# totgokhung123/Event-Retrival-In-Video-Learning-Transferable-Visual-Model-From-Supervised-Natural-Language

Hardware: AMD Instinct MI355X
Metric: frames/sec embedded+ranked, ViT-B/32 224², 1/2/4/8 MI355X; R@1/5/10 parity (higher is better)
Workload: dtype bf16; 1 GPU; ViT-B/32 bf16, 10000 frames/GPU x 32 text queries, top-10 (BASELINE configs[1]); frames_per_gpu=10000, global_frames=10000, queries=32, k=10, image_chunk=10000, parallelism=dp1

## Files before the change

### event-retrival-in-video-learning-transferable-visual-model-from-supervised-natural-language_amd/csrc/api.cpp

```cpp
#include <hip/hip_runtime.h>

#include <cmath>
#include <cstdarg>
#include <cstdlib>
#include <cstdio>
#include <cstring>
#include <algorithm>
#include <functional>
#include <memory>
#include <mutex>
#include <string>
#include <system_error>
#include <thread>
#include <vector>

#include "../../include/miclip.h"
#include "src_hash.h"
#include "internal.hpp"

using namespace miclip;

namespace {

thread_local std::string g_err;
// ... 628 lines not shown
    HIP_TRY(gemm_bf16(with_variant(gargs(c->h, W, L.w_qkv, W, L.b_qkv, c->qkv, 3 * W, M, 3 * W, W), GV_QKV), EPI_BF16,
                      s));
    HIP_TRY(attention(c->qkv, c->att, B, S, W, causal, s));
    HIP_TRY(gemm_bf16(with_variant(gargs(c->att, W, L.w_out, W, L.b_out, c->delta, W, M, W, W), GV_OUT), EPI_BF16, s));
    HIP_TRY(residual_ln(c->x, c->delta, W, 1, L.ln2_g, L.ln2_b, c->h, M, W, s, nullptr, nullptr, xmode_at(r16, l)));
    HIP_TRY(gemm_bf16(with_variant(gargs(c->h, W, L.w_fc, W, L.b_fc, c->mlp, 4 * W, M, 4 * W, W), GV_FC),
                      EPI_GELU_BF16, s));
    HIP_TRY(gemm_bf16(with_variant(gargs(c->mlp, 4 * W, L.w_proj, 4 * W, L.b_proj, c->delta, W, M, W, 4 * W), GV_PROJ),
                      EPI_BF16, s));
    if (l + 1 < layers.size())
      HIP_TRY(residual_ln(c->x, c->delta, W, 1, layers[l + 1].ln1_g, layers[l + 1].ln1_b, c->h, M, W, s, nullptr, nullptr,
                          r16 ? 2 : 0));
  }
  return MI_OK;
}

static int lnfold(int W) { return ab_env_int("MICLIP_LNFOLD", W <= 1024) != 0; }

static GemmArgs ln_args(mi_clip* c, const uint16_t* wf, const float* sv, const float* cv, void* out, int N, int M,
                        int W) {
  GemmArgs g = gargs((const uint16_t*)c->x, 2 * W, wf, W, cv, out, N, M, N, W);
  g.variant = 0;
  g.a_f16 = 1;
  g.rs = c->rs;
  g.colv = sv;
  return g;
}

static int resfuse() { return ab_env_int("MICLIP_RESFUSE", 1) != 0; }

struct Carve {
  char* base;
  size_t cap, off = 0, end = 0;
  void* take(size_t bytes) {
    char* p = base + off;
    end = off + bytes;
    off = (end + 255) & ~(size_t)255;
    return p;
  }
  int fits(const char* what) const {
    return end <= cap ? MI_OK : fail(MI_ERR_ARG, "%s: %zu bytes needed, %zu reserved", what, end, cap);
  }
};
struct ClsRows { void* att; uint8_t* sc; float* x; };
struct RowsOut { char* out; int dtype, l2; };

static int borrow_h(mi_clip* c, size_t bytes, float** p) {
  Carve h{(char*)c->h, c->h_bytes};
  *p = (float*)h.take(bytes);
  return h.fits("rows borrowed from the h buffer");
}

static int gather_rows(void* dst, size_t dst_pitch, const void* src, size_t src_pitch, size_t bytes_per_row, int B,
                       hipStream_t s) {
  HIP_TRY(hipMemcpy2DAsync(dst, dst_pitch, src, src_pitch, bytes_per_row, B, hipMemcpyDeviceToDevice, s));
  return MI_OK;
}

static int gemm_residual(mi_clip* c, const uint16_t* A, int64_t lda, const uint16_t* w, const float* b, float* x, int M,
                         int W, int K, hipStream_t s) {
  GemmArgs g = gargs(A, lda, w, K, b, x, 2 * W, M, W, K);
  MI_TRY(borrow_h(c, (size_t)M * (W / 64) * 8, &g.ps));
  HIP_TRY(gemm_bf16(g, EPI_RES16_BF16, s));
  HIP_TRY(residual_finalize(g.ps, c->rs, M, W, s));
  return MI_OK;
}

static int cls_last() { return ab_env_int("MICLIP_CLS_LAST", 1) != 0; }
static bool cls_att_compact(int S) { return S <= 64 && ab_env_int("MICLIP_CLS_ATT", 1) != 0; }

static bool cls_rows(bool last_layer, int B, int S, bool pre) {
  return last_layer && pre && B >= 256 && S > 1 && cls_last();
}

static int cls_gather(mi_clip* c, int B, int S, int W, const void* att, size_t att_row, const uint8_t* att_sc,
                      size_t x_bytes, hipStream_t s, ClsRows* r, float** xpost, int64_t* post_stride) {
  Carve q{(char*)c->qkv, c->qkv_bytes};
  r->att = q.take(B * att_row);
  r->sc = (uint8_t*)q.take(att_sc ? ((size_t)W / 128) * (B + 2) * 2 : 0);
  r->x = (float*)q.take((size_t)B * W * 4);
  MI_TRY(q.fits("the last block's CLS rows in the qkv buffer"));
  if (att) MI_TRY(gather_rows(r->att, att_row, att, S * att_row, att_row, B, s));
  if (att_sc) {
    const size_t mp = ((size_t)B * S + 1) & ~(size_t)1, bp = ((size_t)B + 1) & ~(size_t)1;
    for (int st = 0; st < W / 128; ++st)
      MI_TRY(gather_rows(r->sc + st * bp * 2, 2, att_sc + st * mp * 2, (size_t)S * 2, 2, B, s));
  }
  MI_TRY(gather_rows(r->x, (size_t)W * 4, c->x, (size_t)S * W * 4, x_bytes, B, s));
  *xpost = r->x;
  *post_stride = 1;
  return MI_OK;
}

using InProjArgs = std::function<GemmArgs(int n0, int N, int rows, int64_t stride)>;
static int in_proj_cls(mi_clip* c, int B, int S, int W, const float* vec, size_t vec_row, const float* GemmArgs::*f,
                       int epi, hipStream_t s, const InProjArgs& mk) {
  float* vec_c;
  MI_TRY(borrow_h(c, B * vec_row, &vec_c));
  HIP_TRY(gemm_bf16(mk(W, 2 * W, B * S, 1), epi, s));
  MI_TRY(gather_rows(vec_c, vec_row, vec, S * vec_row, vec_row, B, s));
  GemmArgs q = mk(0, W, B, S);
  q.*f = vec_c;
  HIP_TRY(gemm_bf16(q, epi, s));
  return MI_OK;
}

static int last_block_cls(mi_clip* c, const Layer& L, int B, int S, int W, bool att_compact, float** xpost,
                          int64_t* post_stride, hipStream_t s) {
  ClsRows r;
  MI_TRY(cls_gather(c, B, S, W, att_compact ? nullptr : c->att, (size_t)W * 2, nullptr, (size_t)W * 2, s, &r, xpost,
                    post_stride));
  if (att_compact) r.att = c->att;
  MI_TRY(gemm_residual(c, (const uint16_t*)r.att, W, L.w_out, L.b_out, r.x, B, W, W, s));
  GemmArgs f = ln_args(c, L.lw_fc, L.ls_fc, L.lc_fc, c->mlp, 4 * W, B, W);
  f.A = (const uint16_t*)r.x;
  HIP_TRY(gemm_bf16(f, EPI_LN_GELU_BF16, s));
  HIP_TRY(gemm_bf16(with_variant(gargs(c->mlp, 4 * W, L.w_proj, 4 * W, L.b_proj, c->delta, W, B, W, 4 * W), GV_PROJ),
                    EPI_BF16, s));
  return MI_OK;
}

static int run_tower_fold(mi_clip* c, const std::vector<Layer>& layers, int B, int S, int W, hipStream_t s,
                          float** xpost, int64_t* post_stride) {
  const int M = B * S;
  const bool fuse = resfuse() && !gemm_variant_for(GV_OUT) && !gemm_variant_for(GV_PROJ) && !gemm_variant();
  *xpost = c->x;
  *post_stride = S;
  for (size_t l = 0; l < layers.size(); ++l) {
    const Layer& L = layers[l];
    const bool last = l + 1 == layers.size();
    const bool cls = cls_rows(last, B, S, fuse);
    auto in_proj = [&](int n0, int N, int rows, int64_t stride) {
      GemmArgs g = ln_args(c, L.lw_qkv + (size_t)n0 * W, L.ls_qkv + n0, L.lc_qkv + n0, c->qkv + n0, N, rows, W);
      g.lda = stride * 2 * W;
      g.ldo = stride * 3 * W;
      return g;
    };
    if (cls) MI_TRY(in_proj_cls(c, B, S, W, c->rs, 8, &GemmArgs::rs, EPI_LN_BF16, s, in_proj));
    else HIP_TRY(gemm_bf16(in_proj(0, 3 * W, M, 1), EPI_LN_BF16, s));
// ... 586 lines not shown
  int r = check_rank_args(N, D, corpus_dtype, Q, 1, norm_mode, MI_NAN_FIRST);
  if (r) return r;
  if (N == 0 || Q == 0) return MI_OK;
  if (!corpus || !queries || !out) return fail(MI_ERR_ARG, "mi_score_matrix: null pointer");
  HIP_TRY(score_matrix(corpus, N, D, corpus_dtype, queries, Q, norm_mode, out, (hipStream_t)stream));
  return MI_OK;
}

int mi_rank_of_targets(const float* scores, int64_t Q, int64_t N, const int64_t* pq, const int64_t* pt, int64_t T,
                       int64_t* out, void* stream) {
  if (Q < 0 || N < 0 || T < 0) return fail(MI_ERR_ARG, "negative size");
  if (T == 0) return MI_OK;
  if (!scores || !pq || !pt || !out) return fail(MI_ERR_ARG, "mi_rank_of_targets: null pointer");
  HIP_TRY(rank_of_targets(scores, Q, N, pq, pt, T, out, (hipStream_t)stream));
  return MI_OK;
}

int mi_op_gemm(const void* A, const void* W, const float* bias, void* out, int32_t M, int32_t N, int32_t K,
               int32_t epi, void* stream) {
  if (!A || !W || !out || M < 0) return fail(MI_ERR_ARG, "mi_op_gemm: bad arguments");
  if (K % 64 || N % 128 || K <= 0) return fail(MI_ERR_UNSUPPORTED, "mi_op_gemm: needs K %% 64 == 0, N %% 128 == 0");
  const int variant = epi >> 8;
  if (variant && !MICLIP_AB) return fail(MI_ERR_UNSUPPORTED, "mi_op_gemm: schedule overrides need the A/B build (make ab)");
  epi &= 0xff;
  if (epi < 0 || epi > 3) return fail(MI_ERR_ARG, "mi_op_gemm: bad epilogue");
  GemmArgs g = gargs((const uint16_t*)A, K, (const uint16_t*)W, K, bias, out, N, M, N, K);
  if (variant) g.variant = variant;
  HIP_TRY(gemm_bf16(g, epi, (hipStream_t)stream));
  return MI_OK;
}

int mi_op_gemm_f32(const float* A, const float* W, const float* bias, float* out, int32_t M, int32_t N, int32_t K,
                   int32_t epi, void* stream) {
  if (!A || !W || !out || M < 0 || N < 1) return fail(MI_ERR_ARG, "mi_op_gemm_f32: bad arguments");
  if (K % 32 || K <= 0) return fail(MI_ERR_UNSUPPORTED, "mi_op_gemm_f32: needs K %% 32 == 0");
  static const int epis[4] = {EPI_F32, EPI_GELU_BF16, EPI_RESID_F32, EPI_RELU_F32};
  if (epi < 0 || epi > 3) return fail(MI_ERR_ARG, "mi_op_gemm_f32: epilogue 0 (store), 1 (QuickGELU), 2 (+=), 3 (ReLU)");
  HIP_TRY(gemm_f32(A, K, W, K, bias, out, N, M, N, K, epis[epi], (hipStream_t)stream));
  return MI_OK;
}

extern "C" int mi_debug_gemm_probe(unsigned long long* host, int32_t n) {
  if (!host || n < 0) return fail(MI_ERR_ARG, "mi_debug_gemm_probe: bad arguments");
  HIP_TRY(gemm_probe_read(host, n));
  return MI_OK;
}

extern "C" int mi_debug_gemm8q_probe(unsigned long long* host, int32_t n) {
  if (!host || n < 0) return fail(MI_ERR_ARG, "mi_debug_gemm8q_probe: bad arguments");
  HIP_TRY(gemm8q_probe_read(host, n));
  return MI_OK;
}

int mi_op_layernorm(const float* x, const float* g, const float* b, void* out, int32_t rows, int32_t W,
                    void* stream) {
  if (!x || !g || !b || !out || rows < 0) return fail(MI_ERR_ARG, "mi_op_layernorm: bad arguments");
  if (W % 4 || W > 1024) return fail(MI_ERR_UNSUPPORTED, "mi_op_layernorm: W must be a multiple of 4, <= 1024");
  HIP_TRY(layernorm_bf16(x, W, g, b, (uint16_t*)out, W, rows, W, (hipStream_t)stream));
  return MI_OK;
}

int mi_op_residual_ln(void* x, const void* delta, const float* g, const float* b, void* out, int32_t rows, int32_t W,
                      int32_t xmode, void* stream) {
  if (!x || !delta || !g || !b || !out || rows < 0) return fail(MI_ERR_ARG, "mi_op_residual_ln: bad arguments");
  if (W % 4 || W > 1024) return fail(MI_ERR_UNSUPPORTED, "mi_op_residual_ln: W must be a multiple of 4, <= 1024");
  if (xmode < 0 || xmode > 2) return fail(MI_ERR_ARG, "mi_op_residual_ln: xmode must be 0, 1 or 2");
  HIP_TRY(residual_ln((float*)x, (const uint16_t*)delta, W, 1, g, b, (uint16_t*)out, rows, W, (hipStream_t)stream,
                      nullptr, nullptr, xmode));
  return MI_OK;
}

int mi_op_split6(const float* x, int64_t ldx, int64_t rows, int32_t K, int32_t role, int32_t gelu, void* out,
                 void* stream) {
  if (!x || !out || rows < 0 || (role & ~1) || (gelu & ~1)) return fail(MI_ERR_ARG, "mi_op_split6: bad arguments");
  if (K < 4 || K % 4 || ldx < K || ldx % 4) return fail(MI_ERR_UNSUPPORTED, "mi_op_split6: K %% 4 == 0, ldx >= K, ldx %% 4 == 0");
  HIP_TRY(split6_rows(x, ldx, rows, K, role, gelu, (uint16_t*)out, (hipStream_t)stream));
  return MI_OK;
}

int mi_clip_kernel_events(mi_clip* c, int32_t kind, int32_t capacity) {
  if (!c || kind < 0 || kind > MI_KERNEL_C_FC || capacity < 0 || capacity > (1 << 16))
    return fail(MI_ERR_ARG, "mi_clip_kernel_events: bad arguments");
  std::lock_guard<std::mutex> g(c->mu);
  HIP_TRY(hipSetDevice(c->device));
  while ((int)c->ev.size() < 2 * capacity) {
    hipEvent_t e;
    HIP_TRY(hipEventCreate(&e));
    c->ev.push_back(e);
  }
  c->ev_kind = capacity ? kind : 0;
  c->ev_cap = capacity;
  c->ev_n = 0;
  return MI_OK;
}

int mi_clip_kernel_times(mi_clip* c, float* us, int32_t n) {
  if (!c || (!us && n > 0) || n < 0) return fail(MI_ERR_ARG, "mi_clip_kernel_times: bad arguments");
  std::lock_guard<std::mutex> g(c->mu);
  const int m = c->ev_n < n ? c->ev_n : n;
  for (int i = 0; i < m; ++i) {
    HIP_TRY(hipEventSynchronize(c->ev[2 * i + 1]));
    float ms = 0.f;
    HIP_TRY(hipEventElapsedTime(&ms, c->ev[2 * i], c->ev[2 * i + 1]));
    us[i] = ms * 1e3f;
  }
  return m;
// ... 256 lines not shown
```

### event-retrival-in-video-learning-transferable-visual-model-from-supervised-natural-language_amd/csrc/encoder.hip

```cpp
#include <cstdlib>

#include "common.hpp"
#include "internal.hpp"

namespace miclip {

namespace {

constexpr float LN_EPS = 1e-5f;

struct RowVals {
  float4 v[4];
};

__device__ __forceinline__ void ln_stats(RowVals& r, int n4, int lane, int W, float& mean, float& rstd) {
  float s = 0.f;
#pragma unroll
  for (int i = 0; i < 4; ++i)
    if (lane + 64 * i < n4) s += (r.v[i].x + r.v[i].y) + (r.v[i].z + r.v[i].w);
  mean = wave_sum(s) / (float)W;
  float ss = 0.f;
#pragma unroll
  for (int i = 0; i < 4; ++i)
    if (lane + 64 * i < n4) {
// ... 150 lines not shown
    ln_stats(r, n4, lane, W, mean, rstd);
    ln_store(r, mean, rstd, g1, b1, h + (int64_t)row * W, nullptr, nullptr, row, 0, lane, n4);
  }
}

__device__ __forceinline__ void store_row_stats(RowVals& r, int n4, int lane, int W, float* rs, int row) {
  float mean, rstd;
  ln_stats(r, n4, lane, W, mean, rstd);
  if (lane == 0) *(float2*)(rs + 2 * (int64_t)row) = make_float2(rstd, rstd * mean);
}

__global__ __launch_bounds__(256) void vision_embed_ln16_kernel(float* __restrict__ x, const float* __restrict__ cls,
                                                                const float* __restrict__ pos,
                                                                const float* __restrict__ g,
                                                                const float* __restrict__ b, int rows, int S, int W,
                                                                float* __restrict__ rs) {
  typedef _Float16 h4v __attribute__((ext_vector_type(4)));
  const int row = blockIdx.x * 4 + (threadIdx.x >> 6), lane = threadIdx.x & 63;
  if (row >= rows) return;
  const int t = row % S, n4 = W >> 2;
  const float4* xr = (const float4*)(x + (int64_t)row * W);
  h4v* xh = (h4v*)((_Float16*)x + (int64_t)row * W * 2);
  const float4* src = t == 0 ? (const float4*)cls : xr;
  const float4* p4 = (const float4*)(pos + (int64_t)t * W);
  RowVals r;
#pragma unroll
  for (int i = 0; i < 4; ++i) {
    const int idx = lane + 64 * i;
    if (idx < n4) {
      const float4 sv = src[idx], p = p4[idx];
      r.v[i] = make_float4(sv.x + p.x, sv.y + p.y, sv.z + p.z, sv.w + p.w);
    } else {
      r.v[i] = make_float4(0.f, 0.f, 0.f, 0.f);
    }
  }
  float mean, rstd;
  ln_stats(r, n4, lane, W, mean, rstd);
  const float4* g4 = (const float4*)g;
  const float4* b4 = (const float4*)b;
#pragma unroll
  for (int i = 0; i < 4; ++i) {
    const int idx = lane + 64 * i;
    if (idx < n4) {
      const float4 gg = g4[idx], bb = b4[idx];
      const h4v o{(_Float16)((r.v[i].x - mean) * rstd * gg.x + bb.x), (_Float16)((r.v[i].y - mean) * rstd * gg.y + bb.y),
                  (_Float16)((r.v[i].z - mean) * rstd * gg.z + bb.z), (_Float16)((r.v[i].w - mean) * rstd * gg.w + bb.w)};
      r.v[i] = make_float4((float)o[0], (float)o[1], (float)o[2], (float)o[3]);
      xh[idx] = o;
    }
  }
  store_row_stats(r, n4, lane, W, rs, row);
}

__global__ __launch_bounds__(256) void residual_stats_kernel(float* __restrict__ x, const uint16_t* __restrict__ delta,
                                                             float* __restrict__ rs, int rows, int W) {
  typedef _Float16 h4v __attribute__((ext_vector_type(4)));
  typedef uint32_t u2v __attribute__((ext_vector_type(2)));
  const int row = blockIdx.x * 4 + (threadIdx.x >> 6), lane = threadIdx.x & 63;
  if (row >= rows) return;
  const int n4 = W >> 2;
  h4v* xh = (h4v*)((_Float16*)x + (int64_t)row * W * 2);
  const u2v* dr = (const u2v*)(delta + (int64_t)row * W);
  RowVals r;
#pragma unroll
  for (int i = 0; i < 4; ++i) {
    const int idx = lane + 64 * i;
    if (idx < n4) {
      const h4v vh = __builtin_nontemporal_load(&xh[idx]);
      const u2v d = __builtin_nontemporal_load(&dr[idx]);
      const h4v o{(_Float16)((float)vh[0] + bf2f((uint16_t)(d[0] & 0xffff))),
                  (_Float16)((float)vh[1] + bf2f((uint16_t)(d[0] >> 16))),
                  (_Float16)((float)vh[2] + bf2f((uint16_t)(d[1] & 0xffff))),
                  (_Float16)((float)vh[3] + bf2f((uint16_t)(d[1] >> 16)))};
      __builtin_nontemporal_store(o, &xh[idx]);
      r.v[i] = make_float4((float)o[0], (float)o[1], (float)o[2], (float)o[3]);
    } else {
      r.v[i] = make_float4(0.f, 0.f, 0.f, 0.f);
    }
  }
  store_row_stats(r, n4, lane, W, rs, row);
}

__global__ __launch_bounds__(256) void residual_finalize_kernel(const float* __restrict__ ps, float* __restrict__ rs,
                                                                int rows, int W) {
  __shared__ float4 sp[256 * 8 + 256 / 4];
  const int np = W >> 6, nq = np >> 1;
  const int r0 = blockIdx.x * 256;
  const int nrow = min(256, rows - r0);
  const float4* src = (const float4*)(ps + (int64_t)r0 * np * 2);
  for (int i = threadIdx.x; i < nrow * nq; i += 256) {
    const int r = i / nq;
    sp[i + (r >> 2)] = src[i];
  }
  __syncthreads();
  const int row = r0 + threadIdx.x;
  if (row >= rows) return;
  const float4* p4 = sp + threadIdx.x * nq + (threadIdx.x >> 2);
  float s[16], m2[16];
#pragma unroll
  for (int i = 0; i < 8; ++i)
    if (i < nq) {
      const float4 v = p4[i];
      s[2 * i] = v.x;
      m2[2 * i] = v.y;
      s[2 * i + 1] = v.z;
      m2[2 * i + 1] = v.w;
    }
  float tot = 0.f;
#pragma unroll
  for (int j = 0; j < 16; ++j)
    if (j < np) tot += s[j];
  const float mean = tot / (float)W;
  float acc = 0.f;
#pragma unroll
  for (int j = 0; j < 16; ++j)
    if (j < np) {
      const float dm = s[j] * (1.0f / 64.0f) - mean;
      acc += m2[j] + 64.0f * dm * dm;
    }
  const float rstd = 1.0f / sqrtf(acc / (float)W + LN_EPS);
  *(float2*)(rs + 2 * (int64_t)row) = make_float2(rstd, rstd * mean);
}

__global__ __launch_bounds__(256) void text_embed_kernel(const int32_t* __restrict__ tokens,
                                                         const float* __restrict__ tok_emb,
                                                         const float* __restrict__ pos, float* __restrict__ x,
                                                         int64_t total4, int S, int W, int vocab) {
  const int64_t i = (int64_t)blockIdx.x * 256 + threadIdx.x;
  if (i >= total4) return;
  const int n4 = W >> 2;
  const int64_t row = i / n4;
  const int c = (int)(i % n4);
  const int t = (int)(row % S);
  int tok = tokens[row];
  tok = tok < 0 ? 0 : (tok >= vocab ? vocab - 1 : tok);
  const float4 e = ((const float4*)(tok_emb + (int64_t)tok * W))[c];
  const float4 p = ((const float4*)(pos + (int64_t)t * W))[c];
  ((float4*)x)[i] = make_float4(e.x + p.x, e.y + p.y, e.z + p.z, e.w + p.w);
}

__global__ __launch_bounds__(256) void eot_gather_ln_kernel(const int32_t* __restrict__ tokens,
                                                            const float* __restrict__ x,
                                                            const uint16_t* __restrict__ delta,
                                                            const float* __restrict__ g,
                                                            const float* __restrict__ b, uint16_t* __restrict__ out,
// ... 72 lines not shown

template <bool IN_BF16>
__global__ __launch_bounds__(256) void im2col_kernel(const void* __restrict__ pixels, uint16_t* __restrict__ out,
                                                     int64_t total8, int R, int P, int G, int Kp) {
  const int64_t i = (int64_t)blockIdx.x * 256 + threadIdx.x;
  if (i >= total8) return;
  const int k8 = Kp >> 3;
  const int64_t prow = i / k8;
  const int kb = (int)(i % k8) * 8;
  const int64_t bimg = prow / (G * G);
  const int p = (int)(prow % (G * G));
  const int gy = p / G, gx = p % G;
  const int PP = P * P, K = 3 * PP;
  uint32_t packed[4];
#pragma unroll
  for (int e = 0; e < 8; e += 2) {
    float v[2];
#pragma unroll
    for (int u = 0; u < 2; ++u) {
      const int k = kb + e + u;
      if (k < K) {
        const int c = k / PP, rem = k % PP, kh = rem / P, kw = rem % P;
        const int64_t off = ((bimg * 3 + c) * R + (gy * P + kh)) * (int64_t)R + gx * P + kw;
        v[u] = IN_BF16 ? bf2f(((const uint16_t*)pixels)[off]) : ((const float*)pixels)[off];
      } else {
        v[u] = 0.f;
      }
    }
    packed[e >> 1] = (uint32_t)f2bf(v[0]) | ((uint32_t)f2bf(v[1]) << 16);
  }
  *(uint4*)(out + prow * Kp + kb) = make_uint4(packed[0], packed[1], packed[2], packed[3]);
}

__global__ __launch_bounds__(256) void finalize_kernel(const float* __restrict__ y, void* __restrict__ out,
                                                       int out_dtype, int rows, int D, int l2) {
  const int row = blockIdx.x * 4 + (threadIdx.x >> 6), lane = threadIdx.x & 63;
  if (row >= rows) return;
  const float* yr = y + (int64_t)row * D;
  float inv = 1.f;
  if (l2) {
    float ss = 0.f;
    for (int c = lane; c < D; c += 64) ss += yr[c] * yr[c];
    const float n = sqrtf(wave_sum(ss));
    inv = (l2 == 2 && !(n > 1e-8f)) ? 1.0f : 1.0f / n;
  }
  for (int c = lane; c < D; c += 64) {
    const float v = l2 ? yr[c] * inv : yr[c];
    if (out_dtype == 0) ((float*)out)[(int64_t)row * D + c] = v;
    else if (out_dtype == 1) ((uint16_t*)out)[(int64_t)row * D + c] = f2bf(v);
    else ((_Float16*)out)[(int64_t)row * D + c] = (_Float16)v;
  }
}

}

hipError_t layernorm_bf16(const float* x, int64_t in_stride, const float* g, const float* b, uint16_t* out,
                          int64_t out_stride, int rows, int W, hipStream_t s, uint8_t* q, uint8_t* qs) {
  if (rows <= 0) return hipSuccess;
  if (W % 4 || W > 1024 || (q && W % 128)) return hipErrorInvalidValue;
  hipLaunchKernelGGL(ln_bf16_kernel, dim3((rows + 3) / 4), dim3(256), 0, s, x, in_stride, g, b, out, out_stride,
                     rows, W, q, qs);
  return hipGetLastError();
}

hipError_t vision_embed_ln(float* x, const float* cls, const float* pos, const float* g, const float* b, int B,
                           int S, int W, hipStream_t s, const float* g1, const float* b1, uint16_t* h) {
  const int rows = B * S;
  if (rows <= 0) return hipSuccess;
  if (W % 4 || W > 1024) return hipErrorInvalidValue;
  hipLaunchKernelGGL(vision_embed_ln_kernel, dim3((rows + 3) / 4), dim3(256), 0, s, x, cls, pos, g, b, rows, S, W,
                     g1, b1, h);
  return hipGetLastError();
}

hipError_t vision_embed_ln16(float* x, const float* cls, const float* pos, const float* g, const float* b, int B,
                             int S, int W, float* rs, hipStream_t s) {
  const int rows = B * S;
  if (W % 4 || W > 1024) return hipErrorInvalidValue;
  if (rows <= 0) return hipSuccess;
  hipLaunchKernelGGL(vision_embed_ln16_kernel, dim3((rows + 3) / 4), dim3(256), 0, s, x, cls, pos, g, b, rows, S, W, rs);
  return hipGetLastError();
}

hipError_t residual_stats(float* x, const uint16_t* delta, float* rs, int rows, int W, hipStream_t s) {
  if (W % 4 || W > 1024) return hipErrorInvalidValue;
  if (rows <= 0) return hipSuccess;
  hipLaunchKernelGGL(residual_stats_kernel, dim3((rows + 3) / 4), dim3(256), 0, s, x, delta, rs, rows, W);
  return hipGetLastError();
}

hipError_t residual_finalize(const float* ps, float* rs, int rows, int W, hipStream_t s) {
  if (W % 128 || W > 1024 || W <= 0) return hipErrorInvalidValue;
  if (rows <= 0) return hipSuccess;
  hipLaunchKernelGGL(residual_finalize_kernel, dim3((rows + 255) / 256), dim3(256), 0, s, ps, rs, rows, W);
  return hipGetLastError();
}

hipError_t text_embed(const int32_t* tokens, const float* tok_emb, const float* pos, float* x, int Q, int S, int W,
                      int vocab, hipStream_t s) {
  const int64_t total4 = (int64_t)Q * S * (W / 4);
  if (total4 <= 0) return hipSuccess;
  hipLaunchKernelGGL(text_embed_kernel, dim3((unsigned)((total4 + 255) / 256)), dim3(256), 0, s, tokens, tok_emb,
                     pos, x, total4, S, W, vocab);
  return hipGetLastError();
}

hipError_t eot_gather_ln(const int32_t* tokens, const float* x, const uint16_t* delta, const float* g,
                         const float* b, uint16_t* out, int Q, int S, int W, hipStream_t s) {
  if (Q <= 0) return hipSuccess;
  hipLaunchKernelGGL(eot_gather_ln_kernel, dim3((Q + 3) / 4), dim3(256), 0, s, tokens, x, delta, g, b, out, Q, S,
                     W);
  return hipGetLastError();
}

hipError_t residual_ln(float* x, const uint16_t* delta, int64_t stride, int write_x, const float* g, const float* b,
                       uint16_t* out, int rows, int W, hipStream_t s, uint8_t* q, uint8_t* qs, int xmode) {
  if (rows <= 0) return hipSuccess;
  if (W % 4 || W > 1024 || (q && W % 128) || xmode < RES_F32 || xmode > RES_F16) return hipErrorInvalidValue;
#if MICLIP_AB
  static int nts = -1;
  if (nts < 0) {
    const char* e = getenv("MICLIP_LN_NT");
    nts = e ? atoi(e) : 1;
  }
#else
  constexpr int nts = 1;
#endif
  const dim3 grid((rows + 3) / 4), block(256);
#define RLN(NT, XM) hipLaunchKernelGGL((residual_ln_kernel<NT, XM>), grid, block, 0, s, x, delta, stride, write_x, g, b, out, rows, W, q, qs)
  if (nts) {
    if (xmode == RES_F32) RLN(true, RES_F32);
    else if (xmode == RES_F32_TO_F16) RLN(true, RES_F32_TO_F16);
    else RLN(true, RES_F16);
  } else {
#if MICLIP_AB
    if (xmode == RES_F32) RLN(false, RES_F32);
    else if (xmode == RES_F32_TO_F16) RLN(false, RES_F32_TO_F16);
    else RLN(false, RES_F16);
#endif
  }
#undef RLN
  return hipGetLastError();
}

hipError_t im2col(const void* pixels, int in_bf16, uint16_t* out, int B, int R, int P, int Kp, hipStream_t s) {
  const int G = R / P;
  const int64_t total8 = (int64_t)B * G * G * (Kp / 8);
  if (total8 <= 0) return hipSuccess;
// ... 21 lines not shown
```

### event-retrival-in-video-learning-transferable-visual-model-from-supervised-natural-language_amd/csrc/gemm.hip

```cpp
#include "gemm_common.hpp"

namespace miclip {

namespace {

constexpr int BK = 32;
constexpr int RING = 4;
constexpr int LEAD = 3;
constexpr int STAGE_OPS = 2 * 2;
static_assert((LEAD - 1) * STAGE_OPS + 16 <= VM_MAX, "counted waits exceed vmcnt's 6-bit field");
constexpr int MAX_N = 4096;
constexpr int EPI_NONE = 9;

__device__ __forceinline__ void split_gelu_store(const GemmArgs& a, int m, int n, float4 v) {
  const float bound = (a.rmax[m] * a.bnd_w + a.bnd_b) * (1.0f + 0.00390625f);
  const int e = split_exp(bound);
  const float y[4] = {quick_gelu_f32(v.x), quick_gelu_f32(v.y), quick_gelu_f32(v.z), quick_gelu_f32(v.w)};
  typedef _Float16 h4 __attribute__((ext_vector_type(4)));
  _Float16 p1[4], p2[4];
#pragma unroll
  for (int i = 0; i < 4; ++i) split2h(ldexpf(y[i], e), p1[i], p2[i]);
  const h4 h1 = {p1[0], p1[1], p1[2], p1[3]}, h2 = {p2[0], p2[1], p2[2], p2[3]};
  _Float16* o = (_Float16*)a.out + (int64_t)m * a.ldo + n;
  const int N = a.N;
// ... 341 lines not shown
        const int r = wr * WTM + mi * 16 + (lane & 15);
        const int c = wc * WTN + ni * 16 + 4 * (lane >> 4);
        *(uint2*)(smem + r * RS + c * 2) = make_uint2(pack_bf16x2(v0, v1), pack_bf16x2(v2, v3));
      }
    __syncthreads();
    constexpr int CH = BN / 8;
#pragma unroll 4
    for (int f = tid; f < BM * CH; f += NT) {
      const int r = f / CH, c8 = f % CH;
      const int m = m0 + r;
      if (m < a.M)
        *(uint4*)((uint16_t*)a.out + out_row(m) * a.ldo + n0 + c8 * 8) = *(const uint4*)(smem + r * RS + c8 * 16);
    }
  } else {
    constexpr int RS = BN * 4 + 16;
    float4 csc[4];
#pragma unroll
    for (int ni = 0; ni < 4; ++ni)
      csc[ni] = F16 ? *(const float4*)(a.csc + n0 + wc * WTN + ni * 16 + 4 * (lane >> 4)) : make_float4(1.f, 1.f, 1.f, 1.f);
#pragma unroll
    for (int p = 0; p < 2; ++p) {
      if (wr == p) {
#pragma unroll
        for (int mi = 0; mi < 8; ++mi) {
          const int mr = min(m0 + wr * WTM + mi * 16 + (lane & 15), a.M - 1);
          const float rs = F16 ? a.rsc[mr] : 1.f;
#pragma unroll
          for (int ni = 0; ni < 4; ++ni) {
            const int r = mi * 16 + (lane & 15);
            const int c = wc * WTN + ni * 16 + 4 * (lane >> 4);
            f32x4 v = acc[mi][ni];
            if (F16) v = v * (f32x4){rs * csc[ni].x, rs * csc[ni].y, rs * csc[ni].z, rs * csc[ni].w};
            *(float4*)(smem + r * RS + c * 4) =
                make_float4(v[0] + bias[ni].x, v[1] + bias[ni].y, v[2] + bias[ni].z, v[3] + bias[ni].w);
          }
        }
      }
      __syncthreads();
      constexpr int C4 = BN / 4;
#pragma unroll 4
      for (int f = tid; f < WTM * C4; f += NT) {
        const int r = f / C4, c4 = f % C4;
        const int m = m0 + p * WTM + r;
        if (m < a.M) {
          const float4 v = *(const float4*)(smem + r * RS + c4 * 16);
          if constexpr (EPI == EPI_SPLIT_GELU) {
            split_gelu_store(a, m, n0 + c4 * 4, v);
            continue;
          }
          float4* dst = (float4*)((float*)a.out + out_row(m) * a.ldo + n0 + c4 * 4);
          if (EPI == EPI_RESID_F32) {
            const float4 o = *dst;
            *dst = make_float4(o.x + v.x, o.y + v.y, o.z + v.z, o.w + v.w);
          } else {
            *dst = v;
          }
        }
      }
      if (p == 0) __syncthreads();
    }
  }
}

template <int ABL>
__global__ __launch_bounds__(512) void gemm_abl_kernel(GemmArgs a) {
  constexpr int BM = 256, BN = 256;
  constexpr int WTM = 128, WTN = 64;
  constexpr int A_BYTES = BM * BK * 2, STAGE_BYTES = (BM + BN) * BK * 2;
  __shared__ __attribute__((aligned(16))) char smem[RING * STAGE_BYTES];
  const int tid = threadIdx.x, lane = tid & 63, wave = tid >> 6;
  const int grp = __builtin_amdgcn_readfirstlane(wave >> 2), wc = wave & 3;
  const int tiles_n = a.N / BN;
  const int tiles_m = (a.M + BM - 1) / BM;
  int m0, n0;
  tile_coords(xcd_remap(blockIdx.x, tiles_m * tiles_n), tiles_m, tiles_n, 0, m0, n0);
  m0 *= BM;
  n0 *= BN;
  const int nk = a.K / BK;
  const int lrow = lane >> 2;
  const int lchunk = ((lane & 3) ^ swz(lane >> 4)) * 8;
  const uint16_t* asrc[2];
  const uint16_t* wsrc[2];
#pragma unroll
  for (int j = 0; j < 2; ++j) {
    asrc[j] = a.A + (int64_t)min(m0 + (wave * 2 + j) * 16 + lrow, a.M - 1) * a.lda + lchunk;
    wsrc[j] = a.W + (int64_t)(n0 + (wave * 2 + j) * 16 + lrow) * a.ldw + lchunk;
  }
  const int frow = lane >> 3, fcol = (lane & 7) * 8;
  auto issue_half = [&](int st, int j) {
    if (ABL == 1) return;
    char* base = smem + (st % RING) * STAGE_BYTES;
    if (ABL == 4 || ABL == 5) {
      const int r0 = (st & 1) * 128 + (wave * 2 + j) * 8 + frow;
      const int64_t k0 = (int64_t)(st >> 1) * 64 + fcol;
      glds16(a.A + (int64_t)min(m0 + r0, a.M - 1) * a.lda + k0, base + (wave * 2 + j) * 1024);
      glds16(a.W + (int64_t)(n0 + r0) * a.ldw + k0, base + A_BYTES + (wave * 2 + j) * 1024);
      return;
    }
    glds16(asrc[j] + (int64_t)st * BK, base + (wave * 2 + j) * 1024);
    glds16(wsrc[j] + st * BK, base + A_BYTES + (wave * 2 + j) * 1024);
  };
  auto wait_stage = [&](int g1) {
    const int younger = min(LEAD - 1, nk - 1 - g1);
    vm_wait_stages<STAGE_OPS, LEAD - 1>(younger);
  };
  auto barrier = [&]() {
// ... 346 lines not shown
      case 70:
        if (bf16_out && gemm_w4_ok(a)) return gemm_w4(a, EPI, s, cus);
        break;
      case 80 ... 86:
      case 89:
        ga.ngroup = v - 80;
        if (bf16_out && gemm_8p_ok(a)) return gemm_8p(ga, EPI, s, cus);
        break;
      case 87 ... 88:
        if (bf16_out && gemm_8p_ok(a)) return gemm_8p(a, EPI, s, cus, v - 80);
        break;
      case 91 ... 94:
      case 96:
        if (bf16_out && gemm_8p_ok(a)) return gemm_8p(a, EPI, s, cus, v - 90);
        break;
      case 97 ... 99:
        if (bf16_out && gemm_8p_ok(a)) return gemm_8p(a, EPI, s, cus, v + 3);
        break;
      case 110 ... 119:
        if (!bf16_out) break;
        if (gemm_8q_ok(a)) return gemm_8q(a, EPI, s, cus, v - 110);
        v = 98;
        continue;
      case 120 ... 124:
        if (!bf16_out) break;
        if (gemm_8r_ok(a)) return gemm_8r(a, EPI, s, cus, v - 120);
        v = 98;
        continue;
      case 125:
        if (bf16_out && gemm_8q_ok(a)) return gemm_8q(a, EPI, s, cus, 10);
        break;
      case 131 ... 139:
        ga.ngroup = v == 131 ? -1 : v - 130;
        if (bf16_out && gemm_8q_ok(a)) return gemm_8q(ga, EPI, s, cus, 0);
        break;
      default:
        break;
    }
    return launch_tiled<EPI>(a, big, s);
  }
}

#endif

template <int EPI>
hipError_t launch(const GemmArgs& a, hipStream_t s) {
  const bool big = a.N % 256 == 0 && a.M >= 1024;
  const bool bf16_out = EPI == EPI_BF16 || EPI == EPI_GELU_BF16;
  const bool staged = big && a.K / BK >= LEAD;
  const int cus = cu_count();
  const int nt = tile_count(a, 256, 256);
  if (a.patch_R) {
    if (!big || a.K != 3 * 32 * 32 || (a.patch_R & 31)) return hipErrorInvalidValue;
    return launch_kernel(gemm_pp_kernel<EPI, 1, false, false, false, true>, nt, 512, s, a);
  }
  if (a.a_f16) {
    if ((EPI != EPI_F32 && EPI != EPI_RESID_F32 && EPI != EPI_SPLIT_GELU) || !a.rsc || !a.csc || a.variant)
      return hipErrorInvalidValue;
    if (EPI == EPI_SPLIT_GELU && (!a.rmax || !a.rsc_out || a.group || a.ldo != (a.o_dup ? 2 : 3) * (int64_t)a.N))
      return hipErrorInvalidValue;
    if constexpr (EPI == EPI_F32 || EPI == EPI_RESID_F32 || EPI == EPI_SPLIT_GELU) {
      const int bit = EPI == EPI_F32 ? 1 : (EPI == EPI_RESID_F32 ? 2 : 4);
      const bool use8q = ab_env_int("MICLIP_F32_8Q", 1) != 0 && (ab_env_int("MICLIP_F32_8Q_MASK", 7) & bit);
      if (use8q && a.bias && gemm_8q_ok(a)) return gemm_8q(a, EPI, s, cus, 0);
      if (a.a_dup || a.o_dup) return hipErrorInvalidValue;
      if (staged) return launch_kernel(gemm_pp_kernel<EPI, 1, false, false, false, false, true>, nt, 512, s, a);
      return launch_tiled<EPI, true>(a, big, s);
    }
    return hipErrorInvalidValue;
  }
#if MICLIP_AB
  if (a.variant != 0) return launch_ab<EPI>(a, s);
#else
  if (a.variant != 0) return hipErrorNotSupported;
#endif
  const int small_t = ab_env_int("MICLIP_SMALLM", 64);
  const int small64 = ab_env_int("MICLIP_SMALL64", cus);
  if (EPI == EPI_BF16 && nt < small_t && a.N % 128 == 0 && !a.group) {
    const int nt2 = tile_count(a, 128, 128);
    if (nt2 < small64)
      return launch_kernel(gemm_kernel<EPI, 64, 64, 2, 2>, persistent_grid(tile_count(a, 64, 64), 4 * cus), 256, s, a);
    return launch_kernel(gemm_kernel<EPI, 128, 128, 2, 2>, persistent_grid(nt2, 2 * cus), 256, s, a);
  }
  if (bf16_out && gemm_8q_ok(a)) return gemm_8q(a, EPI, s, cus, 0);
  if (staged && bf16_out && !a.group && (a.N >= 2048 || a.K <= 1024))
    return launch_kernel(gemm_ppp_kernel<EPI>, persistent_grid(nt, cus), 512, s, a);
  if (staged && bf16_out) return launch_kernel(gemm_pp_kernel<EPI, 1, false, true>, nt, 512, s, a);
  if (staged) return launch_kernel(gemm_pp_kernel<EPI, 1, false>, nt, 512, s, a);
  return launch_tiled<EPI>(a, big, s);
}

}

hipError_t gemm_probe_read(unsigned long long* host, int n) {
#if MICLIP_AB
  if (n > 4096 * 4) n = 4096 * 4;
  return hipMemcpyFromSymbol(host, HIP_SYMBOL(g_gemm_probe), n * sizeof(unsigned long long), 0, hipMemcpyDeviceToHost);
#else
  (void)host;
  (void)n;
  return hipErrorNotSupported;
#endif
}

hipError_t gemm_bf16(const GemmArgs& a, int epi, hipStream_t s) {
  if (a.M <= 0) return hipSuccess;
  if (a.K % BK || a.N % 128 || a.K <= 0 || a.N > MAX_N) return hipErrorInvalidValue;
// ... 18 lines not shown
```

### event-retrival-in-video-learning-transferable-visual-model-from-supervised-natural-language_amd/csrc/internal.hpp

```cpp
#pragma once
#include <hip/hip_runtime.h>
#include <stdint.h>

#include <cstdlib>
#include <type_traits>

#ifndef MICLIP_AB
#define MICLIP_AB 0
#endif

namespace miclip {


template <class... P, class... Args>
hipError_t launch_kernel(void (*kernel)(P...), dim3 grid, int threads, hipStream_t s, const Args&... args) {
  hipLaunchKernelGGL(kernel, grid, dim3(threads), 0, s, args...);
  return hipGetLastError();
}
template <auto KERNEL, class... Args>
hipError_t launch_kernel(int grid, int threads, size_t lds, hipStream_t s, const Args&... args) {
  static bool raised = false;
  if (!raised) {
    const hipError_t e = hipFuncSetAttribute((const void*)KERNEL, hipFuncAttributeMaxDynamicSharedMemorySize, 160 * 1024);
    if (e != hipSuccess) return e;
// ... 104 lines not shown
  int o_dup = 0;
};

hipError_t gemm_bf16(const GemmArgs& a, int epi, hipStream_t s);
int gemm_w4_ok(const GemmArgs& a);
hipError_t gemm_w4(const GemmArgs& a, int epi, hipStream_t s, int cus);
int gemm_8p_ok(const GemmArgs& a);
hipError_t gemm_8p(const GemmArgs& a, int epi, hipStream_t s, int cus, int abl = 0);
int gemm_1d_ok(const GemmArgs& a);
hipError_t gemm_1d(const GemmArgs& a, int abl, hipStream_t s, int cus);
int gemm_8q_ok(const GemmArgs& a);
hipError_t gemm_8q(const GemmArgs& a, int epi, hipStream_t s, int cus, int mode = 0);
hipError_t gemm8q_probe_read(unsigned long long* host, int n);
constexpr int JPEG_LDS_SETS = 4;
struct JpegXform {
  int n, mode, out_bf16;
  void* out;
};
bool jpeg_xform_fits(int H, int W, int n, int mode);
enum JpegGeomSlot {
  JG_W = 0, JG_H = 1, JG_NCOMP = 2,
  JG_RI = 3,
  JG_NSEG = 4,
  JG_HS = 5, JG_VS = 6,
  JG_QSEL = 11,
  JG_DCSEL = 14, JG_ACSEL = 17,
  JG_SLOTS = 20
};
hipError_t jpeg_decode(const uint8_t* data, int64_t data_bytes, const int64_t* seg_off, const int64_t* seg_end,
                       const void* huff, const int32_t* huff_idx, int nsets, const uint16_t* qtab, const int32_t* geom,
                       int nframes, uint8_t* out_rgb, void* ws, size_t ws_bytes, hipStream_t s,
                       const JpegXform* xf = nullptr);
size_t jpeg_workspace_bytes(const int32_t* geom, int nframes, int64_t data_bytes);
int gemm_8r_ok(const GemmArgs& a);
hipError_t gemm_8r(const GemmArgs& a, int epi, hipStream_t s, int cus, int mode = 0);
hipError_t gemm_probe_read(unsigned long long* host, int n);
hipError_t gemm_mx(const GemmArgs& a, int epi, hipStream_t s);
int gemm_mx8q_ok(const GemmArgs& a, int epi);
hipError_t gemm_mx8q(const GemmArgs& a, int epi, hipStream_t s, int cus);
int cu_count();
hipError_t quantize_mx(const uint16_t* in, int64_t ld_in, uint8_t* q, int64_t ld_q, uint8_t* sc, int rows, int K,
                       hipStream_t s);

hipError_t layernorm_bf16(const float* x, int64_t in_stride, const float* g, const float* b,
                          uint16_t* out, int64_t out_stride, int rows, int W, hipStream_t s,
                          uint8_t* q = nullptr, uint8_t* qs = nullptr);
hipError_t vision_embed_ln(float* x, const float* cls, const float* pos, const float* g,
                           const float* b, int B, int S, int W, hipStream_t s, const float* g1 = nullptr,
                           const float* b1 = nullptr, uint16_t* h = nullptr);
hipError_t vision_embed_ln16(float* x, const float* cls, const float* pos, const float* g, const float* b, int B,
                             int S, int W, float* rs, hipStream_t s);
hipError_t residual_stats(float* x, const uint16_t* delta, float* rs, int rows, int W, hipStream_t s);
hipError_t residual_finalize(const float* ps, float* rs, int rows, int W, hipStream_t s);
hipError_t text_embed(const int32_t* tokens, const float* tok_emb, const float* pos, float* x,
                      int Q, int S, int W, int vocab, hipStream_t s);
hipError_t eot_gather_ln(const int32_t* tokens, const float* x, const uint16_t* delta, const float* g,
                         const float* b, uint16_t* out, int Q, int S, int W, hipStream_t s);
hipError_t residual_ln(float* x, const uint16_t* delta, int64_t stride, int write_x, const float* g, const float* b,
                       uint16_t* out, int rows, int W, hipStream_t s, uint8_t* q = nullptr, uint8_t* qs = nullptr,
                       int xmode = 0);
hipError_t im2col(const void* pixels, int in_bf16, uint16_t* out, int B, int R, int P, int Kp,
                  hipStream_t s);
hipError_t attention(const uint16_t* qkv, uint16_t* out, int B, int S, int W, int flags,
                     hipStream_t s, uint8_t* q8 = nullptr, uint8_t* qs = nullptr, uint16_t* cls_out = nullptr,
                     int64_t cls_pitch = 0);
hipError_t finalize_rows(const float* y, void* out, int out_dtype, int rows, int D, int l2,
                         hipStream_t s);

hipError_t gemm_f32(const float* A, int64_t lda, const float* W, int64_t ldw, const float* bias, float* out,
                    int64_t ldo, int M, int N, int K, int epi, hipStream_t s, int group = 0, int gstride = 0,
                    int goffset = 0);
hipError_t layernorm_f32(const float* x, int64_t in_stride, const float* g, const float* b, float* out,
                         int64_t out_stride, int rows, int W, hipStream_t s, const int32_t* tokens = nullptr,
                         int S = 0);
hipError_t attention_f32(const float* qkv, float* out, int B, int S, int W, int causal, hipStream_t s);
hipError_t attention_f32_split(const float* qkv, const float* rmax, float bw, float bb, uint16_t* a3, int role,
                               float* rsc, int B, int S, int W, int causal, hipStream_t s);
hipError_t im2col_f32(const void* pixels, int in_bf16, float* out, int B, int R, int P, int Kp, hipStream_t s);
hipError_t im2col_split2h(const void* pixels, int in_bf16, int B, int R, int P, int Kp, uint16_t* out, float* sc,
                          hipStream_t s);
hipError_t split6_rows(const float* x, int64_t ldx, int64_t rows, int K, int role, int gelu, uint16_t* out,
                       hipStream_t s);
hipError_t split2h_rows(const float* x, int64_t ldx, int64_t rows, int K, int role, int gelu, uint16_t* out,
                        float* sc, hipStream_t s);
hipError_t layernorm_split2h(const float* x, int64_t in_stride, const float* g, const float* b, int rows, int W,
                             uint16_t* out, float* sc, hipStream_t s, float* rmax = nullptr, int dup = 0);

}

namespace miclip {
constexpr int RANK_REG_K = 64;
constexpr int RANK_MAX_K = 1 << 24;
constexpr int RANK_MAX_D = 1024;
size_t rank_workspace_bytes(int64_t N, int64_t Q, int k);
hipError_t rank_topk(const void* corpus, int64_t N, int64_t D, int dt, const float* q, int64_t Q, int k,
                     int64_t base, int norm_mode, int nan_first, float* out_s, int64_t* out_i, void* ws,
                     hipStream_t s);
hipError_t rank_merge(const float* cs, const int64_t* ci, int64_t Q, int64_t C, int k, int nan_first, float* out_s,
                      int64_t* out_i, hipStream_t s);
hipError_t rank_fill_empty(int64_t Q, int k, float* out_s, int64_t* out_i, hipStream_t s);
hipError_t score_matrix(const void* corpus, int64_t N, int64_t D, int dt, const float* q, int64_t Q, int norm_mode,
                        float* out, hipStream_t s);
hipError_t rank_of_targets(const float* S, int64_t Q, int64_t N, const int64_t* pq, const int64_t* pt, int64_t T,
                           int64_t* out, hipStream_t s);
size_t rank_filtered_workspace_bytes(int64_t N, int64_t Q, int k);
int64_t rank_filtered_max_rows(int k);
// ... 63 lines not shown
```

Baseline: 116,300 frames/s.

## Replace strided row gathers with a kernel and batch finalize loads

Strided hipMemcpy2DAsync row gathers are replaced by a custom gather kernel that uses the widest aligned element and handles several segments in one launch, which folds the per-stripe scale gathers into a single launch. residual_finalize is templated on the quarter count so each thread issues its nontemporal loads up front. The patch-embedding GEMM now uses nontemporal stores by default. An experimental multi-row embed+LN kernel sits behind an A/B env flag. Debug entry points are also added.

```diff
diff --git a/event-retrival-in-video-learning-transferable-visual-model-from-supervised-natural-language_amd/csrc/api.cpp b/event-retrival-in-video-learning-transferable-visual-model-from-supervised-natural-language_amd/csrc/api.cpp
--- a/event-retrival-in-video-learning-transferable-visual-model-from-supervised-natural-language_amd/csrc/api.cpp
+++ b/event-retrival-in-video-learning-transferable-visual-model-from-supervised-natural-language_amd/csrc/api.cpp
@@ -704,8 +704,14 @@
 }
 
 static int gather_rows(void* dst, size_t dst_pitch, const void* src, size_t src_pitch, size_t bytes_per_row, int B,
-                       hipStream_t s) {
-  HIP_TRY(hipMemcpy2DAsync(dst, dst_pitch, src, src_pitch, bytes_per_row, B, hipMemcpyDeviceToDevice, s));
+                       hipStream_t s, int nseg = 1, size_t dst_seg = 0, size_t src_seg = 0) {
+  if (ab_env_int("MICLIP_GATHER_COPY", 0) != 0) {
+    for (int g = 0; g < nseg; ++g)
+      HIP_TRY(hipMemcpy2DAsync((char*)dst + g * dst_seg, dst_pitch, (const char*)src + g * src_seg, src_pitch,
+                               bytes_per_row, B, hipMemcpyDeviceToDevice, s));
+    return MI_OK;
+  }
+  HIP_TRY(gather_rows_device(dst, dst_pitch, src, src_pitch, bytes_per_row, B, nseg, dst_seg, src_seg, s));
   return MI_OK;
 }
 
@@ -735,8 +741,7 @@
   if (att) MI_TRY(gather_rows(r->att, att_row, att, S * att_row, att_row, B, s));
   if (att_sc) {
     const size_t mp = ((size_t)B * S + 1) & ~(size_t)1, bp = ((size_t)B + 1) & ~(size_t)1;
-    for (int st = 0; st < W / 128; ++st)
-      MI_TRY(gather_rows(r->sc + st * bp * 2, 2, att_sc + st * mp * 2, (size_t)S * 2, 2, B, s));
+    MI_TRY(gather_rows(r->sc, 2, att_sc, (size_t)S * 2, 2, B, s, W / 128, bp * 2, mp * 2));
   }
   MI_TRY(gather_rows(r->x, (size_t)W * 4, c->x, (size_t)S * W * 4, x_bytes, B, s));
   *xpost = r->x;
@@ -1429,6 +1434,44 @@
   return MI_OK;
 }
 
+extern "C" int mi_debug_vision_embed_ln16(float* x, const float* cls, const float* pos, const float* g, const float* b,
+                                          int32_t B, int32_t S, int32_t W, float* rs, void* stream) {
+  if (!x || !cls || !pos || !g || !b || !rs || B < 0 || S < 1 || W < 4 || (int64_t)B * S > INT32_MAX)
+    return fail(MI_ERR_ARG, "mi_debug_vision_embed_ln16: bad arguments");
+  HIP_TRY(vision_embed_ln16(x, cls, pos, g, b, B, S, W, rs, (hipStream_t)stream));
+  return MI_OK;
+}
+
+extern "C" int mi_debug_residual_finalize(const float* ps, float* rs, int32_t rows, int32_t W, void* stream) {
+  if (!ps || !rs || rows < 0) return fail(MI_ERR_ARG, "mi_debug_residual_finalize: bad arguments");
+  HIP_TRY(residual_finalize(ps, rs, rows, W, (hipStream_t)stream));
+  return MI_OK;
+}
+
+extern "C" int mi_debug_patch_gemm(const void* px, const void* w, float* x, int32_t B, int32_t R, int32_t W,
+                                   void* stream) {
+  if (!px || !w || !x || B < 1 || R < 32 || R % 32 || W < 256) return fail(MI_ERR_ARG, "mi_debug_patch_gemm: bad arguments");
+  const int G2 = (R / 32) * (R / 32);
+  GemmArgs pg = gargs((const uint16_t*)px, 0, (const uint16_t*)w, 3072, nullptr, x, W, B * G2, W, 3072);
+  pg.variant = 0;
+  pg.patch_R = R;
+  pg.group = G2;
+  pg.gstride = G2 + 1;
+  pg.goffset = 1;
+  HIP_TRY(gemm_bf16(pg, EPI_F32, (hipStream_t)stream));
+  return MI_OK;
+}
+
+extern "C" int mi_debug_gather_rows(void* dst, int64_t dst_pitch, const void* src, int64_t src_pitch,
+                                    int64_t bytes_per_row, int32_t B, int32_t nseg, int64_t dst_seg, int64_t src_seg,
+                                    void* stream) {
+  if (!dst || !src || B < 0 || nseg < 1 || bytes_per_row < 0 || dst_pitch < bytes_per_row || src_pitch < bytes_per_row ||
+      dst_seg < 0 || src_seg < 0)
+    return fail(MI_ERR_ARG, "mi_debug_gather_rows: bad arguments");
+  return gather_rows(dst, (size_t)dst_pitch, src, (size_t)src_pitch, (size_t)bytes_per_row, B, (hipStream_t)stream, nseg,
+                     (size_t)dst_seg, (size_t)src_seg);
+}
+
 int mi_op_layernorm(const float* x, const float* g, const float* b, void* out, int32_t rows, int32_t W,
                     void* stream) {
   if (!x || !g || !b || !out || rows < 0) return fail(MI_ERR_ARG, "mi_op_layernorm: bad arguments");
diff --git a/event-retrival-in-video-learning-transferable-visual-model-from-supervised-natural-language_amd/csrc/encoder.hip b/event-retrival-in-video-learning-transferable-visual-model-from-supervised-natural-language_amd/csrc/encoder.hip
--- a/event-retrival-in-video-learning-transferable-visual-model-from-supervised-natural-language_amd/csrc/encoder.hip
+++ b/event-retrival-in-video-learning-transferable-visual-model-from-supervised-natural-language_amd/csrc/encoder.hip
@@ -226,6 +226,66 @@
   store_row_stats(r, n4, lane, W, rs, row);
 }
 
+#if MICLIP_AB
+template <int RPW>
+__global__ __launch_bounds__(256) void vision_embed_ln16_rows_kernel(float* __restrict__ x, const float* __restrict__ cls,
+                                                                     const float* __restrict__ pos,
+                                                                     const float* __restrict__ g,
+                                                                     const float* __restrict__ b, int rows, int S,
+                                                                     int W, float* __restrict__ rs) {
+  typedef _Float16 h4v __attribute__((ext_vector_type(4)));
+  typedef float f4v __attribute__((ext_vector_type(4)));
+  const int row0 = (blockIdx.x * 4 + (threadIdx.x >> 6)) * RPW, lane = threadIdx.x & 63;
+  if (row0 >= rows) return;
+  const int n4 = W >> 2;
+  RowVals r[RPW];
+#pragma unroll
+  for (int j = 0; j < RPW; ++j) {
+    const int row = min(row0 + j, rows - 1);
+    const int t = row % S;
+    const f4v* src = t == 0 ? (const f4v*)cls : (const f4v*)(x + (int64_t)row * W);
+    const float4* p4 = (const float4*)(pos + (int64_t)t * W);
+#pragma unroll
+    for (int i = 0; i < 4; ++i) {
+      const int idx = lane + 64 * i, ic = min(idx, n4 - 1);
+      const f4v sv = __builtin_nontemporal_load(&src[ic]);
+      const float4 p = p4[ic];
+      const float4 v = make_float4(sv[0] + p.x, sv[1] + p.y, sv[2] + p.z, sv[3] + p.w);
+      r[j].v[i] = idx < n4 ? v : make_float4(0.f, 0.f, 0.f, 0.f);
+    }
+  }
+  const float4* g4 = (const float4*)g;
+  const float4* b4 = (const float4*)b;
+  float4 gg[4], bb[4];
+#pragma unroll
+  for (int i = 0; i < 4; ++i) {
+    const int ic = min(lane + 64 * i, n4 - 1);
+    gg[i] = g4[ic];
+    bb[i] = b4[ic];
+  }
+#pragma unroll
+  for (int j = 0; j < RPW; ++j) {
+    const int row = row0 + j;
+    if (row >= rows) break;
+    h4v* xh = (h4v*)((_Float16*)x + (int64_t)row * W * 2);
+    float mean, rstd;
+    ln_stats(r[j], n4, lane, W, mean, rstd);
+#pragma unroll
+    for (int i = 0; i < 4; ++i) {
+      const int idx = lane + 64 * i;
+      const float4 v = r[j].v[i];
+      const h4v o{(_Float16)((v.x - mean) * rstd * gg[i].x + bb[i].x), (_Float16)((v.y - mean) * rstd * gg[i].y + bb[i].y),
+                  (_Float16)((v.z - mean) * rstd * gg[i].z + bb[i].z), (_Float16)((v.w - mean) * rstd * gg[i].w + bb[i].w)};
+      if (idx < n4) {
+        r[j].v[i] = make_float4((float)o[0], (float)o[1], (float)o[2], (float)o[3]);
+        __builtin_nontemporal_store(o, &xh[idx]);
+      }
+    }
+    store_row_stats(r[j], n4, lane, W, rs, row);
+  }
+}
+#endif
+
 __global__ __launch_bounds__(256) void residual_stats_kernel(float* __restrict__ x, const uint16_t* __restrict__ delta,
                                                              float* __restrict__ rs, int rows, int W) {
   typedef _Float16 h4v __attribute__((ext_vector_type(4)));
@@ -255,6 +315,7 @@
   store_row_stats(r, n4, lane, W, rs, row);
 }
 
+template <int NQ>
 __global__ __launch_bounds__(256) void residual_finalize_kernel(const float* __restrict__ ps, float* __restrict__ rs,
                                                                 int rows, int W) {
   __shared__ float4 sp[256 * 8 + 256 / 4];
@@ -262,9 +323,23 @@
   const int r0 = blockIdx.x * 256;
   const int nrow = min(256, rows - r0);
   const float4* src = (const float4*)(ps + (int64_t)r0 * np * 2);
-  for (int i = threadIdx.x; i < nrow * nq; i += 256) {
-    const int r = i / nq;
-    sp[i + (r >> 2)] = src[i];
+  if (NQ > 0) {
+    typedef float f4v __attribute__((ext_vector_type(4)));
+    const f4v* srcv = (const f4v*)src;
+    const int n = nrow * NQ;
+    f4v v[NQ > 0 ? NQ : 1];
+#pragma unroll
+    for (int k = 0; k < NQ; ++k) v[k] = __builtin_nontemporal_load(&srcv[min((int)threadIdx.x + 256 * k, n - 1)]);
+#pragma unroll
+    for (int k = 0; k < NQ; ++k) {
+      const int i = threadIdx.x + 256 * k;
+      if (i < n) sp[i + ((i / NQ) >> 2)] = make_float4(v[k][0], v[k][1], v[k][2], v[k][3]);
+    }
+  } else {
+    for (int i = threadIdx.x; i < nrow * nq; i += 256) {
+      const int r = i / nq;
+      sp[i + (r >> 2)] = src[i];
+    }
   }
   __syncthreads();
   const int row = r0 + threadIdx.x;
@@ -443,6 +518,41 @@
   }
 }
 
+template <class T>
+__global__ __launch_bounds__(256) void gather_rows_kernel(char* __restrict__ dst, int64_t dst_pitch,
+                                                          const char* __restrict__ src, int64_t src_pitch, int ppr,
+                                                          int64_t total, int64_t dst_seg, int64_t src_seg) {
+  const int64_t i = (int64_t)blockIdx.x * 256 + threadIdx.x;
+  if (i >= total) return;
+  const int64_t b = i / ppr;
+  const int64_t c = (i - b * ppr) * (int64_t)sizeof(T);
+  *(T*)(dst + blockIdx.y * dst_seg + b * dst_pitch + c) = *(const T*)(src + blockIdx.y * src_seg + b * src_pitch + c);
+}
+
+}
+
+hipError_t gather_rows_device(void* dst, size_t dst_pitch, const void* src, size_t src_pitch, size_t bytes_per_row,
+                              int B, int nseg, size_t dst_seg, size_t src_seg, hipStream_t s) {
+  if (B <= 0 || bytes_per_row == 0 || nseg <= 0) return hipSuccess;
+  if (nseg > 65535 || bytes_per_row > dst_pitch || bytes_per_row > src_pitch) return hipErrorInvalidValue;
+  const size_t all = (size_t)(uintptr_t)dst | (size_t)(uintptr_t)src | dst_pitch | src_pitch | bytes_per_row |
+                     (nseg > 1 ? dst_seg | src_seg : 0);
+  const int piece = (int)((all & (~all + 1)) < 16 ? (all & (~all + 1)) : 16);
+  const int64_t total = (int64_t)B * (int64_t)(bytes_per_row / piece);
+  if (bytes_per_row / piece > 0x7fffffff || (total + 255) / 256 * 256 * nseg >= ((int64_t)1 << 32)) return hipErrorInvalidValue;
+  const dim3 grid((unsigned)((total + 255) / 256), nseg);
+#define GATHER(T)                                                                                                   \
+  hipLaunchKernelGGL(gather_rows_kernel<T>, grid, dim3(256), 0, s, (char*)dst, (int64_t)dst_pitch, (const char*)src, \
+                     (int64_t)src_pitch, (int)(bytes_per_row / piece), total, (int64_t)dst_seg, (int64_t)src_seg)
+  switch (piece) {
+    case 16: GATHER(uint4); break;
+    case 8: GATHER(uint2); break;
+    case 4: GATHER(uint32_t); break;
+    case 2: GATHER(uint16_t); break;
+    default: GATHER(uint8_t); break;
+  }
+#undef GATHER
+  return hipGetLastError();
 }
 
 hipError_t layernorm_bf16(const float* x, int64_t in_stride, const float* g, const float* b, uint16_t* out,
@@ -469,6 +579,18 @@
   const int rows = B * S;
   if (W % 4 || W > 1024) return hipErrorInvalidValue;
   if (rows <= 0) return hipSuccess;
+#if MICLIP_AB
+  const int rpw = ab_env_int("MICLIP_EMBED16", 0);
+  if (rpw) {
+    const hipError_t e = with_value<1, 2, 4>(rpw, [&](auto n) {
+      constexpr int RPW = decltype(n)::value;
+      hipLaunchKernelGGL(vision_embed_ln16_rows_kernel<RPW>, dim3((rows + 4 * RPW - 1) / (4 * RPW)), dim3(256), 0, s, x,
+                         cls, pos, g, b, rows, S, W, rs);
+      return hipGetLastError();
+    });
+    return e;
+  }
+#endif
   hipLaunchKernelGGL(vision_embed_ln16_kernel, dim3((rows + 3) / 4), dim3(256), 0, s, x, cls, pos, g, b, rows, S, W, rs);
   return hipGetLastError();
 }
@@ -483,8 +605,17 @@
 hipError_t residual_finalize(const float* ps, float* rs, int rows, int W, hipStream_t s) {
   if (W % 128 || W > 1024 || W <= 0) return hipErrorInvalidValue;
   if (rows <= 0) return hipSuccess;
-  hipLaunchKernelGGL(residual_finalize_kernel, dim3((rows + 255) / 256), dim3(256), 0, s, ps, rs, rows, W);
-  return hipGetLastError();
+  const dim3 grid((rows + 255) / 256);
+#if MICLIP_AB
+  if (ab_env_int("MICLIP_FINALIZE_BATCH", 1) == 0) {
+    hipLaunchKernelGGL(residual_finalize_kernel<0>, grid, dim3(256), 0, s, ps, rs, rows, W);
+    return hipGetLastError();
+  }
+#endif
+  return with_value<1, 2, 3, 4, 5, 6, 7, 8>(W >> 7, [&](auto nq) {
+    hipLaunchKernelGGL(residual_finalize_kernel<decltype(nq)::value>, grid, dim3(256), 0, s, ps, rs, rows, W);
+    return hipGetLastError();
+  });
 }
 
 hipError_t text_embed(const int32_t* tokens, const float* tok_emb, const float* pos, float* x, int Q, int S, int W,
diff --git a/event-retrival-in-video-learning-transferable-visual-model-from-supervised-natural-language_amd/csrc/gemm.hip b/event-retrival-in-video-learning-transferable-visual-model-from-supervised-natural-language_amd/csrc/gemm.hip
--- a/event-retrival-in-video-learning-transferable-visual-model-from-supervised-natural-language_amd/csrc/gemm.hip
+++ b/event-retrival-in-video-learning-transferable-visual-model-from-supervised-natural-language_amd/csrc/gemm.hip
@@ -417,6 +417,8 @@
           if (EPI == EPI_RESID_F32) {
             const float4 o = *dst;
             *dst = make_float4(o.x + v.x, o.y + v.y, o.z + v.z, o.w + v.w);
+          } else if (NTS) {
+            __builtin_nontemporal_store((f32x4){v.x, v.y, v.z, v.w}, (f32x4*)dst);
           } else {
             *dst = v;
           }
@@ -869,7 +871,11 @@
   const int nt = tile_count(a, 256, 256);
   if (a.patch_R) {
     if (!big || a.K != 3 * 32 * 32 || (a.patch_R & 31)) return hipErrorInvalidValue;
-    return launch_kernel(gemm_pp_kernel<EPI, 1, false, false, false, true>, nt, 512, s, a);
+#if MICLIP_AB
+    if (ab_env_int("MICLIP_PATCH_NT", 1) == 0)
+      return launch_kernel(gemm_pp_kernel<EPI, 1, false, false, false, true>, nt, 512, s, a);
+#endif
+    return launch_kernel(gemm_pp_kernel<EPI, 1, false, false, true, true>, nt, 512, s, a);
   }
   if (a.a_f16) {
     if ((EPI != EPI_F32 && EPI != EPI_RESID_F32 && EPI != EPI_SPLIT_GELU) || !a.rsc || !a.csc || a.variant)
diff --git a/event-retrival-in-video-learning-transferable-visual-model-from-supervised-natural-language_amd/csrc/internal.hpp b/event-retrival-in-video-learning-transferable-visual-model-from-supervised-natural-language_amd/csrc/internal.hpp
--- a/event-retrival-in-video-learning-transferable-visual-model-from-supervised-natural-language_amd/csrc/internal.hpp
+++ b/event-retrival-in-video-learning-transferable-visual-model-from-supervised-natural-language_amd/csrc/internal.hpp
@@ -180,6 +180,8 @@
                              int S, int W, float* rs, hipStream_t s);
 hipError_t residual_stats(float* x, const uint16_t* delta, float* rs, int rows, int W, hipStream_t s);
 hipError_t residual_finalize(const float* ps, float* rs, int rows, int W, hipStream_t s);
+hipError_t gather_rows_device(void* dst, size_t dst_pitch, const void* src, size_t src_pitch, size_t bytes_per_row,
+                              int B, int nseg, size_t dst_seg, size_t src_seg, hipStream_t s);
 hipError_t text_embed(const int32_t* tokens, const float* tok_emb, const float* pos, float* x,
                       int Q, int S, int W, int vocab, hipStream_t s);
 hipError_t eot_gather_ln(const int32_t* tokens, const float* x, const uint16_t* delta, const float* g,
```

Result: no change. 116,300 frames/s, median of 2 (+0.1%).
